# CliMA/ClimateParameterizations.jl

Hardware: AMD Instinct MI355X
Metric: column-timesteps/sec (fwd+adjoint), 32-level wind-mixing NDE (higher is better)
Workload: dtype f32

## Files before the change

### climateparameterizations.jl_amd/csrc/engine_regtile.hip

```cpp
#include <cstdlib>
#include "engine_regtile.h"
#include "kernel_select.h"
#include "split_bf16.h"

typedef float f32x16 __attribute__((ext_vector_type(16)));

#ifdef COLNDE_STAMPS
__device__ unsigned long long g_rt_stamps[16];
#define RT_STAMP_DECL unsigned long long rs_t0 = 0, rs_acc[8] = {0, 0, 0, 0, 0, 0, 0, 0}; const unsigned long long rs_kk = __builtin_amdgcn_s_memtime(), rs_rr = __builtin_amdgcn_s_memrealtime()
#define RT_STAMP_BEGIN() do { __builtin_amdgcn_sched_barrier(0); rs_t0 = __builtin_amdgcn_s_memtime(); __builtin_amdgcn_sched_barrier(0); } while (0)
#define RT_STAMP(i) do { __builtin_amdgcn_sched_barrier(0); unsigned long long t_ = __builtin_amdgcn_s_memtime(); rs_acc[i] += t_ - rs_t0; rs_t0 = t_; __builtin_amdgcn_sched_barrier(0); } while (0)
#define RT_STAMP_FLUSH() do { if (blockIdx.x == 0 && threadIdx.x == 0) { for (int q_ = 0; q_ < 8; q_++) g_rt_stamps[q_] = rs_acc[q_]; g_rt_stamps[8] = __builtin_amdgcn_s_memtime() - rs_kk; g_rt_stamps[9] = __builtin_amdgcn_s_memrealtime() - rs_rr; } } while (0)
#else
#define RT_STAMP_DECL
#define RT_STAMP_BEGIN()
#define RT_STAMP(i)
#define RT_STAMP_FLUSH()
#endif
typedef float f32x4v __attribute__((ext_vector_type(4)));
typedef float f32x2v __attribute__((ext_vector_type(2)));

#define RHO0(r) (((r) & 3) + 8 * ((r) >> 2))
#ifndef RT16_WAVES
#define RT16_WAVES 8
#endif
#ifndef RT_ADJ_CH
#define RT_ADJ_CH 8
#endif
#ifndef RT_ZRICH
#define RT_ZRICH 0
#endif
#ifndef RT_Z2TAPE
#define RT_Z2TAPE 0
#endif
#define RT_TAPEZ_HALF (21 * 256)
#define RT_Z2OFF ((RT_ZRICH ? 2 : 1) * RT_TAPEZ_HALF)
#define RT_TAPEZ (RT_Z2OFF + (RT_Z2TAPE ? 9 * 256 : 0))
#define RT_TAPE2 (20 * 256)

__device__ __forceinline__ f32x16 mfma32(float a, float b, f32x16 c) {
    return __builtin_amdgcn_mfma_f32_32x32x2f32(a, b, c, 0, 0, 0);
}

__device__ __forceinline__ float xchg32(float from_hi, float from_lo, int h) {
    const auto r = __builtin_amdgcn_permlane32_swap(__float_as_uint(from_hi), __float_as_uint(from_lo), false, false);
    return __uint_as_float(h ? r[0] : r[1]);
}
__device__ __forceinline__ float swap32(float x, int h) { return xchg32(x, x, h); }

__device__ __forceinline__ f32x16 shift_down(const f32x16 T, int h, float below) {
    f32x16 o;
#pragma unroll
    for (int g = 0; g < 4; g++) {
        const float recv = xchg32(g > 0 ? T[(4 * g + 15) & 15] : 0.0f, T[4 * g + 3], h);
        o[4 * g] = (h == 0 && g == 0) ? below : recv;
        o[4 * g + 1] = T[4 * g];
        o[4 * g + 2] = T[4 * g + 1];
        o[4 * g + 3] = T[4 * g + 2];
    }
    return o;
}

__device__ __forceinline__ f32x16 shift_up(const f32x16 T, int h, float above) {
    f32x16 o;
#pragma unroll
    for (int g = 0; g < 4; g++) {
        const float recv = xchg32(T[4 * g], g < 3 ? T[(4 * g + 4) & 15] : 0.0f, h);
        o[4 * g + 3] = (h == 1 && g == 3) ? above : recv;
        o[4 * g] = T[4 * g + 1];
        o[4 * g + 1] = T[4 * g + 2];
        o[4 * g + 2] = T[4 * g + 3];
    }
    return o;
}

template <int ACT>
__device__ __forceinline__ float rt_act(float z) {
    if (ACT == COLNDE_ACT_RELU) return fmaxf(z, 0.0f);
    if (ACT == COLNDE_ACT_MISH) {
        const float e = __expf(__builtin_amdgcn_fmed3f(z, -3.0e38f, 20.0f));
        const float n = e * (e + 2.0f);
        return z * fast_div(n, n + 2.0f);
    }
    if (ACT == COLNDE_ACT_SWISH) return fast_div(z, 1.0f + __expf(-z));
    if (ACT == COLNDE_ACT_TANH) { const float e = __expf(2.0f * fminf(fmaxf(z, -15.0f), 15.0f)); return 1.0f - fast_div(2.0f, 1.0f + e); }
    if (ACT == COLNDE_ACT_LEAKYRELU) return z > 0.0f ? z : 0.01f * z;
    return z;
}

template <int ACT>
__device__ __forceinline__ f32x16 act_tile(f32x16 z) {
    f32x16 o;
#pragma unroll
    for (int r = 0; r < 16; r++) o[r] = rt_act<ACT>(z[r]);
    return o;
}

struct RtBases {
    int a1[5];
    int a2;
    int a3;
};

__device__ __forceinline__ RtBases rt_bases(int lane) {
    const int i = lane & 31, h = lane >> 5;
    const int r_i = (i & 3) + 4 * (i >> 3), h_i = (i >> 2) & 1;
    RtBases b;
#pragma unroll
    for (int mt = 0; mt < 5; mt++) {
        const int G = min(mt * 16 + r_i, 74);
// ... 513 lines not shown
    float av, dv;
    rt_act_pair<ACT>(A[G >> 4][G & 15], av, dv);
    A[G >> 4][G & 15] = av;
    D[G >> 4][G & 15] = dv;
}

__device__ __forceinline__ void rt_physics_vjp(const DevModel& m, const f32x16 (&X)[3], f32x16 (&kd)[3], int h, f32x16 (&xb)[3]) {
    const float Nz = 32.0f;
#pragma unroll
    for (int r = 0; r < 16; r++) {
        xb[0][r] = -m.cor_v * m.sig_u * kd[1][r];
        xb[1][r] = m.cor_u * m.sig_v * kd[0][r];
        xb[2][r] = 0.0f;
    }
#pragma unroll
    for (int k = 0; k < 3; k++) {
        const f32x16 dn = shift_down(kd[k], h, 0.0f);
#pragma unroll
        for (int r = 0; r < 16; r++) kd[k][r] = (r == 0 && h == 0) ? 0.0f : m.A[k] * (kd[k][r] - dn[r]);
    }
    if (!m.mpp && !m.ca) return;
    f32x16 gb[3];
    if (m.mpp) {
        const f32x16 Ud = shift_down(X[0], h, 0.0f), Vd = shift_down(X[1], h, 0.0f), Td = shift_down(X[2], h, 0.0f);
        const float cU = m.sig_u * Nz, sU = m.sig_u * m.eps, cV = m.sig_v * Nz, sV = m.sig_v * m.eps, cB = m.B * Nz, sB = m.B * m.eps;
        const float L2E = 1.4426950408889634f;
        const float kE = 2.0f * m.inv_dRi * L2E, oE = -2.0f * m.Ric * m.inv_dRi * L2E, cE = 30.0f * L2E;
        const float nA = -0.5f * m.nu_minus, nB = m.nu0 + 0.5f * m.nu_minus;
        const float m0 = -m.cs[0], m1 = -m.cs[1], m2 = -m.cs[2] * m.inv_Pr;
        const float n0 = m0 * Nz * m.c_rib, n1 = m1 * Nz * m.c_rib, n2 = m2 * Nz * m.c_rib;
        const float q0 = -2.0f * m.sig_u, q1 = -2.0f * m.sig_v;
#pragma unroll
        for (int r = 0; r < 16; r++) {
            const bool in = !(r == 0 && h == 0);
            const float dU = X[0][r] - Ud[r], dV = X[1][r] - Vd[r], dT = X[2][r] - Td[r];
            const float a1 = fmaf(dU, cU, sU), a2 = fmaf(dV, cV, sV);
            const float rS = __builtin_amdgcn_rcpf(fmaf(a2, a2, a1 * a1));
            const float Ri = fmaf(dT, cB, sB) * rS;
            const float e = __builtin_amdgcn_exp2f(__builtin_amdgcn_fmed3f(fmaf(Ri, kE, oE), -cE, cE));
            const float th = fmaf(-2.0f, __builtin_amdgcn_rcpf(1.0f + e), 1.0f);
            const float nu = fmaf(th, nA, nB);
            const float t0 = kd[0][r] * nu, t1 = kd[1][r] * nu, t2 = kd[2][r] * nu;
            float nub = (kd[0][r] * dU) * n0;
            nub = fmaf(kd[1][r] * dV, n1, nub);
            nub = fmaf(kd[2][r] * dT, n2, nub);
            const float w = nub * (fmaf(-th, th, 1.0f) * rS);
            const float qq = w * Ri;
            const float g2 = fmaf(w, m.B, t2 * m2);
            const float g0 = fmaf(qq, a1 * q0, t0 * m0);
            const float g1 = fmaf(qq, a2 * q1, t1 * m1);
            gb[0][r] = in ? g0 : 0.0f;
            gb[1][r] = in ? g1 : 0.0f;
            gb[2][r] = in ? g2 : 0.0f;
        }
    } else {
        const f32x16 Td = shift_down(X[2], h, 0.0f);
#pragma unroll
        for (int r = 0; r < 16; r++) {
            const bool in = !(r == 0 && h == 0);
            const float gT = (X[2][r] - Td[r]) * Nz;
            gb[0][r] = 0.0f;
            gb[1][r] = 0.0f;
            gb[2][r] = (in && gT < 0.0f) ? -kd[2][r] * m.cs[2] * m.kappa : 0.0f;
        }
    }
#pragma unroll
    for (int k = 0; k < 3; k++) {
        const f32x16 gu_ = shift_up(gb[k], h, 0.0f);
#pragma unroll
        for (int r = 0; r < 16; r++) xb[k][r] += (gb[k][r] - gu_[r]) * Nz;
    }
}

#define RT_DMA_AUX 2
#ifdef RT_PLAIN_TAPE_STORES
#define RT_NT_STORE4(p, v) (*reinterpret_cast<f32x4v*>(p) = (f32x4v)(v))
#define RT_NT_STORE1(p, v) (*(float*)(p) = (float)(v))
#else
#define RT_NT_STORE4(p, v) __builtin_nontemporal_store((f32x4v)(v), reinterpret_cast<f32x4v*>(p))
#define RT_NT_STORE1(p, v) __builtin_nontemporal_store((float)(v), (float*)(p))
#endif
#define RT_TAPE_LOAD4(p) __builtin_nontemporal_load(reinterpret_cast<const f32x4v*>(p))
#define RT_TB (32 * 36)
#define RT_LAM(e, lane) ((((e) >> 2) * 64 + (lane)) * 4 + ((e) & 3))
__device__ __forceinline__ f32x16 rt_transpose(float* tb, const f32x16 T, int wbase, int rbase) {
#pragma unroll
    for (int a = 0; a < 4; a++)
        *reinterpret_cast<f32x4v*>(tb + wbase + 8 * a) = (f32x4v){T[4 * a], T[4 * a + 1], T[4 * a + 2], T[4 * a + 3]};
    f32x16 o;
#pragma unroll
    for (int s = 0; s < 16; s++) o[s] = tb[rbase + 72 * s];
    return o;
}

__device__ __forceinline__ f32x16 rt_outer(f32x16 acc, const f32x16 TA, const f32x16 TB) {
#pragma unroll
    for (int s = 0; s < 16; s++) acc = mfma32(TA[s], TB[s], acc);
    return acc;
}

struct Bf3x2 { Bf3 b[2]; };
__device__ __forceinline__ Bf3x2 rt_split_tile(const f32x16 T) {
    Bf3x2 o;
#pragma unroll
    for (int b = 0; b < 2; b++) {
        float v[8];
#pragma unroll
        for (int u = 0; u < 8; u++) v[u] = T[8 * b + u];
        o.b[b] = bf3_split8(v);
    }
    return o;
}
__device__ __forceinline__ f32x16 rt_outer_split(f32x16 acc, const Bf3x2& A, const Bf3x2& B) {
    acc = mfma_bf3(A.b[0], B.b[0], acc);
    acc = mfma_bf3(A.b[1], B.b[1], acc);
    return acc;
}

__device__ __forceinline__ float rt_sum16(const f32x16 v) {
    float s = 0.0f;
#pragma unroll
    for (int r = 0; r < 16; r++) s += v[r];
    return s;
}

#define RT_NET_LO(mt) (((mt) * 16) / 25)
#define RT_NET_HI(mt) ((((mt) * 16 + 15) < 75 ? ((mt) * 16 + 15) : 74) / 25)
__host__ __device__ constexpr int rt_combo(int n, int mt) { return n == 0 ? mt : (n == 1 ? 1 + mt : 2 + mt); }

template <int ACT, bool ZT, bool SPLIT = false>
__global__ void __launch_bounds__(256)
rt_adjoint_kernel(DevModel m, const float* __restrict__ wimg, const float* __restrict__ bcs,
                  const float* __restrict__ save_times, int n_save, int substeps, const float* __restrict__ sol,
                  const float* __restrict__ truth, const float* __restrict__ tape, float* __restrict__ tape2,
                  const float* __restrict__ tapez ,
                  LossWeights lw, float* __restrict__ slab, int n_col) {
    static_assert(!SPLIT || ZT, "the split W1^T operands replace the fp32 W1 in LDS: no layer-1 recomputation");
    float* wl = rt_smem;
    if constexpr (SPLIT) {
        static_assert(RT_ASIMG_HM_WORDS + 576 <= RT_W2C, "the split W1^T operands must fit the fp32 W1's place");
        const u32x4* src = reinterpret_cast<const u32x4*>(wimg + RT_ASIMG_OFF);
        for (int e = threadIdx.x; e < (RT_ASIMG_HM_WORDS + 576) / 4; e += blockDim.x) reinterpret_cast<u32x4*>(rt_smem)[e] = src[e];
        for (int e = RT_W2C + threadIdx.x; e < RT_IMG_FLOATS; e += blockDim.x) wl[e] = wimg[e];
    } else {
        for (int e = threadIdx.x; e < RT_IMG_FLOATS; e += blockDim.x) wl[e] = wimg[e];
    }
    __syncthreads();
    const int lane = threadIdx.x & 63, wave = threadIdx.x >> 6;
    const int j = lane & 31, h = lane >> 5;
    const int tile = blockIdx.x * RT_WAVES + wave;
    if (tile * RT_COLS >= n_col) return;
    float* lam = rt_smem + ((RT_IMG_FLOATS + 3) & ~3) + wave * (3072 + RT_TB);
    float* tb = lam + 3072;
    const int col = tile * RT_COLS + j;
    const bool valid = col < n_col;
    const int i_ = lane & 31, r_i = (i_ & 3) + 4 * (i_ >> 3), h_i = (i_ >> 2) & 1;
    int a1n[2];
#pragma unroll
    for (int t = 0; t < 2; t++) a1n[t] = RT_W1C + (2 * min(t * 16 + r_i, 24) + h_i) * RT_LD1 + 4 * h;
    const int a2b = RT_W2C + ((r_i < 10) ? 2 * r_i + h_i : 0) * RT_LD2 + h;
    const int f2c = (r_i < 10) ? 2 * r_i + h_i : 20;
    const int b3T = RT_W3C + (4 * h - 1) * RT_LD3 + f2c;
    int b2T[2];
#pragma unroll
    for (int t = 0; t < 2; t++) b2T[t] = RT_W2C + h * RT_LD2 + ((t * 16 + r_i < 25) ? 2 * (t * 16 + r_i) + h_i : 50);
    const int b1T = RT_W1C + h * RT_LD1 + i_;
    const int wbase = j * 36 + 4 * h, rbase = h * 36 + i_;

    f32x16 gW3[3], gW2[3][2];
#pragma unroll
    for (int q = 0; q < 3; q++) { gW3[q] = (f32x16)(0.0f); gW2[q][0] = (f32x16)(0.0f); gW2[q][1] = (f32x16)(0.0f); }
    float b2acc[3] = {0, 0, 0}, b3acc[3] = {0, 0, 0};
    float sums[6] = {0, 0, 0, 0, 0, 0};
    RT_STAMP_DECL;
    f32x16 xb[3], X[3];
#pragma unroll
    for (int q = 0; q < 3; q++) xb[q] = (f32x16)(0.0f);
    f32x16 xbs[3];
#pragma unroll
    for (int q = 0; q < 3; q++) xbs[q] = (f32x16)(0.0f);
#pragma unroll
    for (int e = 0; e < 48; e++) lam[RT_LAM(e, lane)] = 0.0f;

    const int n_steps = (n_save - 1) * substeps;
    const float* tp = tape + (size_t)tile * n_steps * 4 * 3072 + lane * 4;
    float* tp2 = tape2 + (size_t)tile * n_steps * 4 * RT_TAPE2 + lane * 4;
    const float* tpz = ZT ? tapez + (size_t)tile * n_steps * 4 * RT_TAPEZ + lane * 4 : nullptr;

    auto inject = [&](int n, bool add) {
#pragma unroll
        for (int q = 0; q < 3; q++) {
            f32x16 d;
#pragma unroll
            for (int g = 0; g < 4; g++) {
                const size_t o = ((size_t)min(col, n_col - 1) * n_save + n) * 96 + q * 32 + 8 * g + 4 * h;
                const f32x4v a = *reinterpret_cast<const f32x4v*>(sol + o);
                const f32x4v b = *reinterpret_cast<const f32x4v*>(truth + o);
#pragma unroll
                for (int e = 0; e < 4; e++) d[4 * g + e] = valid ? a[e] - b[e] : 0.0f;
            }
            const f32x16 dd = shift_down(d, h, 0.0f);
            f32x16 gg;
#pragma unroll
            for (int r = 0; r < 16; r++) {
                gg[r] = (r == 0 && h == 0) ? 0.0f : (d[r] - dd[r]) * 32.0f;
                sums[q] += d[r] * d[r];
                sums[3 + q] += gg[r] * gg[r];
            }
            if (add) {
                const f32x16 gu_ = shift_up(gg, h, 0.0f);
#pragma unroll
                for (int r = 0; r < 16; r++)
                    lam[RT_LAM(q * 16 + r, lane)] += 2.0f * lw.w[q] * d[r] + 2.0f * lw.w[3 + q] * 32.0f * (gg[r] - gu_[r]);
            }
        }
    };
    inject(0, false);

    auto load_z1 = [&](int step, int st, int n, f32x16 (&Z)[2], f32x16 (&Dz)[2]) {
        size_t rec = (size_t)step * 4 + st;
#ifdef RT_ABL_Z1_CACHED
        { int z_ = 0; asm volatile("" : "+v"(z_)); rec = (size_t)z_; }
#endif
        const float* srcz = tpz + rec * RT_TAPEZ + n * 7 * 256;
#pragma unroll
        for (int grp = 0; grp < 7; grp++) {
            const f32x4v v = RT_TAPE_LOAD4(srcz + grp * 256);
#pragma unroll
            for (int e = 0; e < 4; e++)
                if (4 * grp + e < 25) Z[grp >> 2][(grp & 3) * 4 + e] = v[e];
        }
        if (RT_ZRICH) {
#pragma unroll
            for (int grp = 0; grp < 7; grp++) {
                const f32x4v v = RT_TAPE_LOAD4(srcz + RT_TAPEZ_HALF + grp * 256);
#pragma unroll
                for (int e = 0; e < 4; e++)
                    if (4 * grp + e < 25) Dz[grp >> 2][(grp & 3) * 4 + e] = v[e];
            }
        }
    };

    auto load_z2 = [&](int step, int st, int n, f32x16& Z) {
        const float* srcz = tpz + ((size_t)step * 4 + st) * RT_TAPEZ + RT_Z2OFF + n * 3 * 256;
#pragma unroll
        for (int grp = 0; grp < 3; grp++) {
            const f32x4v v = RT_TAPE_LOAD4(srcz + grp * 256);
#pragma unroll
            for (int e = 0; e < 4; e++) Z[4 * grp + e] = (4 * grp + e < 10) ? v[e] : 0.0f;
        }
#pragma unroll
        for (int r = 12; r < 16; r++) Z[r] = 0.0f;
    };

    auto load_x = [&](int step, int st) {
        const float* src = tp + ((size_t)step * 4 + st) * 3072;
#pragma unroll
        for (int q = 0; q < 3; q++)
#pragma unroll
            for (int g = 0; g < 4; g++) {
                const f32x4v v = RT_TAPE_LOAD4(src + (q * 4 + g) * 256);
                X[q][4 * g] = v[0]; X[q][4 * g + 1] = v[1]; X[q][4 * g + 2] = v[2]; X[q][4 * g + 3] = v[3];
            }
    };

    for (int iv = n_save - 2; iv >= 0; iv--) {
        const float dt = (save_times[iv + 1] - save_times[iv]) / (float)substeps;
        inject(iv + 1, true);
        for (int s = substeps - 1; s >= 0; s--) {
            const int step = iv * substeps + s;
#pragma nounroll
            for (int st = 3; st >= 0; st--) {
                const float cwl = (st == 0 || st == 3) ? dt / 6.0f : dt / 3.0f;
                const float cwx = st == 3 ? 0.0f : (st == 2 ? dt : 0.5f * dt);
                RT_STAMP_BEGIN();
                f32x16 A1[2], D1[2];
                f32x16 A1n[2], D1n[2];
#pragma unroll
                for (int r = 9; r < 16; r++) { A1[1][r] = 0.0f; D1[1][r] = 0.0f; A1n[1][r] = 0.0f; D1n[1][r] = 0.0f; }
                load_x(step, st);
                f32x16 dOk[3];
                {
                    f32x16 kb[3];
#pragma unroll
                    for (int q = 0; q < 3; q++)
#pragma unroll
                        for (int r = 0; r < 16; r++) kb[q][r] = cwl * lam[RT_LAM(q * 16 + r, lane)] + cwx * xb[q][r];
                    rt_physics_vjp(m, X, kb, h, xb);
#pragma unroll
                    for (int q = 0; q < 3; q++) dOk[q] = kb[q];
                }
                RT_STAMP(0);
                float* dst = tp2 + ((size_t)step * 4 + st) * RT_TAPE2;
                float carry[2] = {0.0f, 0.0f};
#pragma unroll
                for (int n = 0; n < 3; n++) {
                    const f32x16 dOn = dOk[n];
                    if (ZT) {
                        if (n == 0) {
                            load_z1(step, st, 0, A1, D1);
#ifdef COLNDE_STAMPS
                            asm volatile("s_waitcnt vmcnt(0)" ::: "memory");
                            RT_STAMP(7);
#endif
                            if (!RT_ZRICH) {
#pragma unroll
                                for (int G = 0; G < 24; G += 4) rt_act_pair4_at<ACT>(A1, D1, G);
                                rt_act_pair_at<ACT>(A1, D1, 24);
                            }
                        }
                    } else {
#pragma unroll
                        for (int t = 0; t < 2; t++) {
                            f32x16 acc;
#pragma unroll
                            for (int r = 0; r < 16; r++) acc[r] = (t * 16 + r < 25) ? wl[RT_B1C + n * 50 + 2 * (t * 16 + r) + h] : 0.0f;
                            const int base = a1n[t] + n * 50 * RT_LD1;
                            acc = rt_chain<48, RT_ADJ_CH>(wl, acc, [=](int k) { return base + (k >> 4) * 32 + RHO0(k & 15); },
                                                          [&](int k) { return X[k >> 4][k & 15]; });
#pragma unroll
                            for (int r = 0; r < 16; r++) {
                                float av = 0.0f, dv = 0.0f;
                                if (t * 16 + r < 25) rt_act_pair<ACT>(acc[r], av, dv);
                                A1[t][r] = av;
                                D1[t][r] = dv;
                            }
                        }
                    }
                    RT_STAMP(1);
                    f32x16 Z2;
                    if (ZT && RT_Z2TAPE) load_z2(step, st, n, Z2);
                    else {
                        f32x16 acc;
#pragma unroll
                        for (int r = 0; r < 16; r++) acc[r] = r < 10 ? wl[RT_B2C + n * 20 + 2 * r + h] : 0.0f;
                        const int base2 = a2b + n * 20 * RT_LD2;
                        Z2 = rt_chain<25, 5>(wl, acc, [=](int k) { return base2 + 2 * k; },
                                             [&](int k) { return A1[k >> 4][k & 15]; });
                    }
                    RT_STAMP(2);
                    {
#ifndef RT_ABL_NO_OUTER
                        const f32x16 TA = rt_transpose(tb, dOn, wbase, rbase);
                        b3acc[n] += rt_sum16(TA);
#endif
                        f32x16 A2;
#pragma unroll
                        for (int r = 0; r < 16; r += 4) {
                            f32x2v a0 = {0.0f, 0.0f}, d0 = {0.0f, 0.0f}, a1 = {0.0f, 0.0f}, d1 = {0.0f, 0.0f};
                            if (r < 8) rt_act_pair4<ACT>((f32x2v){Z2[r], Z2[r + 1]}, (f32x2v){Z2[r + 2], Z2[r + 3]}, a0, d0, a1, d1);
                            else if (r == 8) rt_act_pair2<ACT>((f32x2v){Z2[8], Z2[9]}, a0, d0);
                            A2[r] = a0.x; A2[r + 1] = a0.y; A2[r + 2] = a1.x; A2[r + 3] = a1.y;
                            Z2[r] = d0.x; Z2[r + 1] = d0.y; Z2[r + 2] = d1.x; Z2[r + 3] = d1.y;
                        }
#ifndef RT_ABL_NO_OUTER
                        const f32x16 TB = rt_transpose(tb, A2, wbase, rbase);
#ifdef RT_OUTER_SPLIT
                        if constexpr (SPLIT) gW3[n] = rt_outer_split(gW3[n], rt_split_tile(TA), rt_split_tile(TB));
                        else
#endif
                        gW3[n] = rt_outer(gW3[n], TA, TB);
#else
                        gW3[n][0] += A2[0];
#endif
                    }
                    {
                        const int base = b3T + n * 31 * RT_LD3;
                        const f32x16 da = rt_chain<16, 8>(wl, (f32x16)(0.0f), [=](int k) { return base + RHO0(k) * RT_LD3; },
                                                          [&](int k) { return dOn[k]; });
#pragma unroll
                        for (int r = 0; r < 16; r++) Z2[r] = da[r] * Z2[r];
                    }
                    RT_STAMP(3);
                    if (ZT && n < 2) load_z1(step, st, n + 1, A1n, D1n);
#ifndef RT_LPIPE
#define RT_LPIPE 1
#endif
                    u32x4 Lr[9];
                    const u32x4* lg = nullptr;
                    if constexpr (SPLIT) {
                        int lz = lane;
                        asm volatile("" : "+v"(lz));
                        lg = reinterpret_cast<const u32x4*>(wimg + RT_ASIMG_OFF + RT_ASIMG_L) + n * 9 * 64 + lz;
#pragma unroll
                        for (int u = 0; u < (RT_LPIPE ? 3 : 9); u++) Lr[u] = lg[u * 64];
                    }
#ifdef RT_ABL_NO_OUTER
                    gW2[n][0][0] += Z2[0] * A1[0][0]; gW2[n][1][0] += Z2[1] * A1[1][0];
#else
                    {
                        const f32x16 TA = rt_transpose(tb, Z2, wbase, rbase);
                        b2acc[n] += rt_sum16(TA);
#ifdef RT_OUTER_SPLIT
                        Bf3x2 TAs;
                        if constexpr (SPLIT) TAs = rt_split_tile(TA);
#endif
#pragma unroll
                        for (int t = 0; t < 2; t++) {
                            const f32x16 TB = rt_transpose(tb, A1[t], wbase, rbase);
#ifdef RT_OUTER_SPLIT
                            if constexpr (SPLIT) gW2[n][t] = rt_outer_split(gW2[n][t], TAs, rt_split_tile(TB));
                            else
#endif
                            gW2[n][t] = rt_outer(gW2[n][t], TA, TB);
                        }
                    }
#endif
                    RT_STAMP(4);
#pragma unroll
                    for (int t = 0; t < 2; t++) {
                        const int base = b2T[t] + n * 20 * RT_LD2;
                        const f32x16 da = rt_chain<10, 10>(wl, (f32x16)(0.0f), [=](int k) { return base + 2 * k * RT_LD2; },
                                                           [&](int k) { return Z2[k]; });
#pragma unroll
                        for (int r = 0; r < 16; r++) D1[t][r] = da[r] * D1[t][r];
                    }
                    auto store_delta = [&] {
#pragma unroll
                    for (int g = 0; g < 25; g++) {
                        const int G = 25 * n + g;
                        if ((G & 3) == 0 && g + 3 < 25) {
                            const f32x4v v = {D1[g >> 4][g & 15], D1[(g + 1) >> 4][(g + 1) & 15], D1[(g + 2) >> 4][(g + 2) & 15],
                                              D1[(g + 3) >> 4][(g + 3) & 15]};
                            RT_NT_STORE4(dst + (G >> 2) * 256, v);
                        }
                    }
                    if (n == 0) carry[0] = D1[1][8];
                    if (n == 1) {
                        RT_NT_STORE4(dst + 6 * 256, ((f32x4v){carry[0], D1[0][0], D1[0][1], D1[0][2]}));
                        carry[0] = D1[1][7];
                        carry[1] = D1[1][8];
                    }
                    if (n == 2) {
                        RT_NT_STORE4(dst + 12 * 256, ((f32x4v){carry[0], carry[1], D1[0][0], D1[0][1]}));
                        RT_NT_STORE4(dst + 18 * 256, ((f32x4v){D1[1][6], D1[1][7], D1[1][8], 0.0f}));
                    }
                    };
#ifndef RT_ABL_NO_TAPE2
                    if constexpr (!SPLIT) store_delta();
#endif
                    RT_STAMP(5);
                    if constexpr (SPLIT) {
                        const u32x4* hm = reinterpret_cast<const u32x4*>(rt_smem) + lane;
#pragma unroll
                        for (int c = 0; c < 3; c++) {
                            if (RT_LPIPE && c < 2) {
#pragma unroll
                                for (int u = 0; u < 3; u++) Lr[3 * (c + 1) + u] = lg[(3 * (c + 1) + u) * 64];
                            }
                            float d8[8];
#pragma unroll
                            for (int u = 0; u < 8; u++) d8[u] = D1[(8 * c + u) >> 4][(8 * c + u) & 15];
                            const Bf3 Bc = bf3_split8(d8);
#pragma unroll
                            for (int q = 0; q < 3; q++) {
                                const int G = n * 9 + c * 3 + q, slot = c * 3 + q;
                                const u32x4 Ah = hm[(G * 2) * 64], Am = hm[(G * 2 + 1) * 64];
                                if (ZT && !RT_ZRICH && n < 2 && slot >= 2) {
                                    if (slot < 8) rt_act_pair4_at<ACT>(A1n, D1n, 4 * (slot - 2));
                                    else rt_act_pair_at<ACT>(A1n, D1n, 24);
                                }
                                xb[q] = mfma_bf(Am, Bc.m, xb[q]);
                                xb[q] = mfma_bf(Ah, Bc.l, xb[q]);
                                xb[q] = mfma_bf(Am, Bc.h, xb[q]);
                                xb[q] = mfma_bf(Ah, Bc.m, xb[q]);
                                xb[q] = mfma_bf(Ah, Bc.h, xb[q]);
                                xb[q] = mfma_bf(Lr[slot], Bc.h, xb[q]);
                                RT_SCHED_FENCE();
                            }
                        }
                        const float* left = rt_smem + RT_ASIMG_LEFT + (n * 2 + h) * 96 + i_;
#pragma unroll
                        for (int q = 0; q < 3; q++) xb[q] = mfma32(left[q * 32], D1[1][8], xb[q]);
                        store_delta();
                    } else
#pragma unroll
                    for (int q = 0; q < 3; q++) {
                        const int base = b1T + q * 32 + n * 50 * RT_LD1;
                        xb[q] = rt_chain_fill<25, 5>(wl, xb[q], [=](int g) { return base + 2 * g * RT_LD1; },
                                                     [&](int g) { return D1[g >> 4][g & 15]; },
                                                     [&](int c) {
                                                         if (ZT && !RT_ZRICH && n < 2 && (q > 0 || c > 0)) {
#pragma unroll
                                                             for (int G = 0; G < 24; G += 4)
                                                                 if ((G >> 2) * 2 + 2 == q * 5 + c)
                                                                     rt_act_pair4_at<ACT>(A1n, D1n, G);
                                                             if (q * 5 + c == 14) rt_act_pair_at<ACT>(A1n, D1n, 24);
                                                         }
                                                     });
                    }
                    if (ZT && n < 2) {
#pragma unroll
                        for (int t = 0; t < 2; t++) { A1[t] = A1n[t]; D1[t] = D1n[t]; }
                    }
                }
                RT_STAMP(6);
#pragma unroll
                for (int q = 0; q < 3; q++) xbs[q] += xb[q];
            }
#pragma unroll
            for (int q = 0; q < 3; q++) {
#pragma unroll
                for (int r = 0; r < 16; r++) lam[RT_LAM(q * 16 + r, lane)] += xbs[q][r];
                xbs[q] = (f32x16)(0.0f);
            }
        }
    }

#ifndef COLNDE_STAMPS_FWD
    RT_STAMP_FLUSH();
#endif
    float* out = slab + (size_t)tile * (m.n_params + 8);
    const int r_j = (j & 3) + 4 * (j >> 3), h_j = (j >> 2) & 1;
#pragma unroll
    for (int n = 0; n < 3; n++) {
        if (r_j < 10) {
            const int f2 = 2 * r_j + h_j;
#pragma unroll
            for (int r = 0; r < 16; r++) {
                const int face = RHO0(r) + 4 * h;
                if (face >= 1) out[n * m.net_size + m.w_off[2] + f2 * 31 + face - 1] = gW3[n][r];
            }
        }
#pragma unroll
        for (int t = 0; t < 2; t++) {
            const int Gp = t * 16 + r_j;
            if (Gp < 25) {
                const int f1 = 2 * Gp + h_j;
#pragma unroll
                for (int r = 0; r < 10; r++) out[n * m.net_size + m.w_off[1] + f1 * 20 + 2 * r + h] = gW2[n][t][r];
            }
        }
        const float s2 = b2acc[n] + swap32(b2acc[n], h), s3 = b3acc[n] + swap32(b3acc[n], h);
        if (h == 0) {
            if (r_i < 10) out[n * m.net_size + m.b_off[1] + 2 * r_i + h_i] = s2;
            if (i_ >= 1) out[n * m.net_size + m.b_off[2] + i_ - 1] = s3;
        }
    }
#pragma unroll
    for (int q = 0; q < 6; q++) {
        float v = sums[q];
        for (int off = 32; off > 0; off >>= 1) v += __shfl_down(v, off);
        if (lane == 0) out[m.n_params + q] = v;
    }
}

#define RT_DW1_LDS (4 * 2048)
__global__ void __launch_bounds__(256)
rt_dw1_kernel(DevModel m, const float* __restrict__ tape, const float* __restrict__ tape2, long n_items,
              float* __restrict__ slab_rows) {
    const int lane = threadIdx.x & 63, wave = __builtin_amdgcn_readfirstlane(threadIdx.x >> 6);
    const int j = lane & 31, h = lane >> 5;
    float* buf = rt_smem + wave * RT_DW1_LDS;
    const long gw = (long)blockIdx.x * RT_WAVES + wave, GW = (long)gridDim.x * RT_WAVES;
    f32x16 gW1[5][3];
#pragma unroll
    for (int mt = 0; mt < 5; mt++)
#pragma unroll
        for (int q = 0; q < 3; q++) gW1[mt][q] = (f32x16)(0.0f);
    float b1acc[5] = {0, 0, 0, 0, 0};
    const int NQ = gw < n_items ? 4 * (int)((n_items - gw + GW - 1) / GW) : 0;
    const int soff = ((lane >> 1) & 3) * 256 + ((lane & 1) * 32 + (lane >> 3)) * 4;
    auto issue = [&](int Q, int ring) {
        const int Qc = Q < NQ ? Q : NQ - 1;
        const size_t item = (size_t)(gw + (long)(Qc >> 2) * GW);
        const float* sx = tape + item * 3072 + soff + (Qc & 3) * 32;
        const float* sz = tape2 + item * RT_TAPE2 + soff + (Qc & 3) * 32;
#pragma unroll
        for (int T = 0; T < 3; T++) __builtin_amdgcn_global_load_lds(sx + T * 1024, buf + ring * 2048 + T * 256, 16, 0, RT_DMA_AUX);
#pragma unroll
        for (int T = 0; T < 5; T++) __builtin_amdgcn_global_load_lds(sz + T * 1024, buf + ring * 2048 + (3 + T) * 256, 16, 0, RT_DMA_AUX);
    };
    const float* rd = buf + h * 32 + j;
    float op[2][8][4];
    auto read_set = [&](int set, int ring) {
#pragma unroll
        for (int T = 0; T < 8; T++)
#pragma unroll
            for (int s = 0; s < 4; s++) op[set][T][s] = rd[ring * 2048 + T * 256 + 64 * s];
    };
    if (NQ > 0) {
        issue(0, 0);
        issue(1, 1);
        issue(2, 2);
        asm volatile("s_waitcnt vmcnt(16)" ::: "memory");
        read_set(0, 0);
    }
    for (int Qb = 0; Qb < NQ; Qb += 4) {
#pragma unroll
        for (int u = 0; u < 4; u++) {
            const int cur = u & 1;
// ... 2091 lines not shown
                    for (int i = 0; i < 11; i++) *reinterpret_cast<f32x4v*>(rec + rec_wr[i]) = *reinterpret_cast<const f32x4v*>(stg + stg_rd[i]);
                }
#pragma unroll
                for (int t = 0; t < 4; t++) gb1[t] += dZ1[t];
#pragma unroll
                for (int u = 0; u < 2; u++) { gb2[u] += dZ2[u]; gb3[u] += dO.t[u]; }
                RT_STAMP(3);
                if constexpr (SPLIT) {
                    const float d80[8] = {dZ1[0][0], dZ1[0][1], dZ1[0][2], dZ1[0][3], dZ1[1][0], dZ1[1][1], dZ1[1][2], dZ1[1][3]};
                    const float d81[8] = {dZ1[2][0], dZ1[2][1], dZ1[2][2], dZ1[2][3], dZ1[3][0], dZ1[3][1], dZ1[3][2], dZ1[3][3]};
                    const Bf3 B0 = bf3_split8(d80);
                    Bf3 B1 = B0;
                    f32x4t c2[6];
#pragma unroll
                    for (int tl = 0; tl < 6; tl++) {
                        Bf3 A0;
                        A0.h = Hm[tl * 2 + 0]; A0.m = Hm[tl * 2 + 1]; A0.l = Lr[tl];
                        c2[tl] = mfma16_bf3(A0, B0, (f32x4t)(0.0f));
                        RT_SCHED_FENCE();
                        if (tl < 4) {
                            bf3_split_pair(d81[2 * tl], d81[2 * tl + 1], tl, B1);
                            RT_SCHED_FENCE();
                        }
                    }
#pragma unroll
                    for (int tl = 0; tl < 6; tl++) {
                        Bf3 A1_;
                        A1_.h = Hm[(6 + tl) * 2 + 0]; A1_.m = Hm[(6 + tl) * 2 + 1]; A1_.l = Lr[6 + tl];
                        c2[tl] = mfma16_bf3(A1_, B1, c2[tl]);
                        ex[(n * 6 + tl) * 64 + lane] = c2[tl];
                        RT_SCHED_FENCE();
                    }
                } else
#pragma unroll
                for (int q = 0; q < 3; q++) {
                    if (q < 2) rt16_fetch_ops<2, 13>(wl, a1[(q + 1) & 1], [&](int c, int k) { return b1T + 32 * (q + 1) + 16 * c + 4 * k * RT_LD1; });
                    RT_SCHED_HARD();
                    f32x4t c2[2] = {(f32x4t)(0.0f), (f32x4t)(0.0f)};
                    rt16_run_ops<2, 13>(a1[q & 1], c2, [&](int k) { return dZ1[k >> 2][k & 3]; });
#pragma unroll
                    for (int tau = 0; tau < 2; tau++) ex[(n * 6 + q * 2 + tau) * 64 + lane] = c2[tau];
                    RT_SCHED_HARD();
                }
                RT_STAMP(4);
                asm volatile("s_waitcnt lgkmcnt(0)\n\ts_barrier" ::: "memory");
                RT_STAMP(5);
            }
        }
    }
#ifndef COLNDE_STAMPS_FWD
    RT_STAMP_FLUSH();
#endif
    auto colsum = [&](float v) {
        v += __shfl_xor(v, 1); v += __shfl_xor(v, 2); v += __shfl_xor(v, 4); v += __shfl_xor(v, 8);
        return v;
    };
#pragma unroll
    for (int Q = 0; Q < 13; Q++) {
        const float v = colsum(gb1[Q >> 2][Q & 3]);
        if (j == 0 && (Q < 12 || g < 2)) out[n * m.net_size + m.b_off[0] + 4 * Q + g] = v;
    }
#pragma unroll
    for (int Q2 = 0; Q2 < 5; Q2++) {
        const float v = colsum(gb2[Q2 >> 2][Q2 & 3]);
        if (j == 0) out[n * m.net_size + m.b_off[1] + 4 * Q2 + g] = v;
    }
#pragma unroll
    for (int v_ = 0; v_ < 2; v_++)
#pragma unroll
        for (int r = 0; r < 4; r++) {
            const float v = colsum(gb3[v_][r]);
            const int face = 16 * v_ + 4 * g + r;
            if (j == 0 && face >= 1) out[n * m.net_size + m.b_off[2] + face - 1] = v;
        }
}

bool rt_supported(const DevModel& m) {
    return m.model == COLNDE_MODEL_WIND_MIXING && m.Nz == 32 && m.n_layers == 3 && m.sizes[0] == 96 && m.sizes[1] == 50 &&
           m.sizes[2] == 20 && m.sizes[3] == 31 && m.acts[0] == m.acts[1] && m.acts[2] == COLNDE_ACT_IDENTITY &&
           !m.smooth_NN && !m.smooth_Ri && !m.inplace;
}

size_t rt_forward_lds_bytes() { return (size_t)RT_IMG_FLOATS * sizeof(float); }
size_t rt_adjoint_lds_bytes() { return ((size_t)((RT_IMG_FLOATS + 3) & ~3) + RT_WAVES * (3072 + RT_TB)) * sizeof(float); }
static constexpr size_t rt_pad4(size_t floats) { return (floats + 3) & ~(size_t)3; }
static constexpr size_t RT_IMG_BYTES = rt_pad4(RT_IMG_FLOATS) * sizeof(float);
static constexpr size_t RT16S_FWD_XCH = 3 * 2 * 64 * 16;
static constexpr size_t RT16S_ADJ_XCH = 3 * 6 * 64 * 16;
static constexpr size_t RT16S_ADJ_STG = 3 * RT16S_STG * sizeof(float);
static size_t rt16_forward_lds_bytes(bool split) { return split ? ((size_t)RT_SIMG_WORDS + (RT_IMG_FLOATS - RT_B1C)) * sizeof(float) : rt_forward_lds_bytes(); }
static size_t rt16s_forward_lds_bytes() { return RT_IMG_BYTES + 2 * RT16S_FWD_XCH; }
static size_t rt16sh_forward_lds_bytes(bool split) {
    return (split ? ((size_t)RT_SIMG2_WORDS + rt_pad4(RT_IMG_FLOATS - RT_W3C)) * sizeof(float) : RT_IMG_BYTES) + 3 * RT16S_FWD_XCH;
}
static size_t rt16s_adjoint_lds_bytes() { return RT_IMG_BYTES + 2 * RT16S_ADJ_XCH + RT16S_ADJ_STG; }
static size_t rt16sh_adjoint_lds_bytes(bool split) {
    const size_t rest = RT16S_ADJ_XCH + 3 * 2 * 64 * 16 + RT16S_ADJ_STG;
    return split ? rt_pad4(RT_IMG_FLOATS - RT_W2C) * sizeof(float) + rest + (size_t)RT_NSA_HM_WORDS * 4 : RT_IMG_BYTES + rest;
}
static size_t rt_dw1_lds_bytes() { return RT_WAVES * RT_DW1_LDS * sizeof(float); }
size_t rt_tape_floats(int n_col, int n_steps) { return (size_t)((n_col + RT_COLS - 1) / RT_COLS) * n_steps * 4 * 3072; }
size_t rt_tape2_floats(int n_col, int n_steps) { return (size_t)((n_col + RT_COLS - 1) / RT_COLS) * n_steps * 4 * RT_TAPE2; }
size_t rt_split_rich_record_floats() { return RT16S_RREC; }
size_t rt_tapez_floats(int n_col, int n_steps) { return (size_t)((n_col + RT_COLS - 1) / RT_COLS) * n_steps * 4 * RT_TAPEZ; }
int rt_n_wtiles(int n_col) { return (n_col + RT_COLS - 1) / RT_COLS; }
int rt_dw1_waves(int n_col, int n_steps) {
    const long items = (long)rt_n_wtiles(n_col) * n_steps * 4;
    const long w = items < 1024 ? items : 1024;
    return (int)((w + RT_WAVES - 1) / RT_WAVES) * RT_WAVES;
}

using RtForwardFn = decltype(&rt_forward_kernel<COLNDE_ACT_RELU>);
using Rt16ForwardFn = decltype(&rt16_forward_kernel<COLNDE_ACT_RELU, false>);
using Rt16sForwardFn = decltype(&rt16s_forward_kernel<COLNDE_ACT_RELU, false>);
using Rt16shForwardFn = decltype(&rt16sh_forward_kernel<COLNDE_ACT_RELU, false>);
using Rt16sAdjointFn = decltype(&rt16s_adjoint_kernel<COLNDE_ACT_RELU, false>);
using Rt16shAdjointFn = decltype(&rt16sh_adjoint_kernel<COLNDE_ACT_RELU, false>);
using RtAdjointFn = decltype(&rt_adjoint_kernel<COLNDE_ACT_RELU, false>);

static RtForwardFn rt_forward_pick(int act) {
    RtForwardFn k = nullptr;
    with_act(act, [&](auto A) { k = rt_forward_kernel<decltype(A)::value>; });
    return k;
}
static Rt16ForwardFn rt16_forward_pick(int act, bool split) {
    Rt16ForwardFn k = nullptr;
    with_act(act, [&](auto A) { with_bools([&](auto S) { k = rt16_forward_kernel<decltype(A)::value, decltype(S)::value>; }, split); });
    return k;
}
static Rt16sForwardFn rt16s_forward_pick(int act, bool rich) {
    Rt16sForwardFn k = nullptr;
    with_act(act, [&](auto A) { with_bools([&](auto R) { k = rt16s_forward_kernel<decltype(A)::value, decltype(R)::value>; }, rich); });
    return k;
}
static Rt16shForwardFn rt16sh_forward_pick(int act, bool rich, bool rkc, bool split) {
    Rt16shForwardFn k = nullptr;
    with_act(act, [&](auto A) {
        with_bools([&](auto R, auto K, auto S) { k = rt16sh_forward_kernel<decltype(A)::value, decltype(R)::value, decltype(K)::value, decltype(S)::value>; }, rich, rkc, split);
    });
    return k;
}
static Rt16sAdjointFn rt16s_adjoint_pick(int act, bool rich) {
    Rt16sAdjointFn k = nullptr;
    with_act(act, [&](auto A) { with_bools([&](auto R) { k = rt16s_adjoint_kernel<decltype(A)::value, decltype(R)::value>; }, rich); });
    return k;
}
static Rt16shAdjointFn rt16sh_adjoint_pick(int act, bool rich, bool rkc, bool split) {
    Rt16shAdjointFn k = nullptr;
    with_act(act, [&](auto A) {
        with_bools([&](auto R, auto K, auto S) { k = rt16sh_adjoint_kernel<decltype(A)::value, decltype(R)::value, decltype(K)::value, decltype(S)::value>; }, rich, rkc, split);
    });
    return k;
}
static RtAdjointFn rt_adjoint_pick(int act, bool ztape, bool split) {
    RtAdjointFn k = nullptr;
    with_act(act, [&](auto A) {
        with_bools([&](auto Z, auto S) {
            if constexpr (decltype(Z)::value || !decltype(S)::value) k = rt_adjoint_kernel<decltype(A)::value, decltype(Z)::value, decltype(S)::value>;
        }, ztape, split);
    });
    return k;
}
static auto rt_dw1_pick(bool split) { return split ? rt_dw1_split_kernel : rt_dw1_kernel; }

hipError_t rt_set_attributes() {
    hipError_t e = hipSuccess;
    const size_t v = 160 * 1024;
// ... 128 lines not shown
```

Before: 185.2 million.

## Stream Z1 tape records into LDS via async global_load_lds ring with vmcnt pacing

Replaces the register-destined nontemporal loads of the layer-1 Z tape in the adjoint kernel with asynchronous global-to-LDS DMA (global_load_lds). Four groups go to a per-wave LDS ring and the rest into the transposition tile. Waits on vmcnt are placed so the loads for the next record overlap the current chain computation. This is meant to hide tape-load latency and free VGPRs, at the cost of extra LDS per wave (a static assert checks the 160KB fit), a possible occupancy reduction, and fragile hand-counted vmcnt thresholds.

Result: no change. 186.4 million (median of 6 runs) (+0.7%).

```diff
diff --git a/climateparameterizations.jl_amd/csrc/engine_regtile.hip b/climateparameterizations.jl_amd/csrc/engine_regtile.hip
--- a/climateparameterizations.jl_amd/csrc/engine_regtile.hip
+++ b/climateparameterizations.jl_amd/csrc/engine_regtile.hip
@@ -26,6 +26,9 @@
 #endif
 #ifndef RT_ADJ_CH
 #define RT_ADJ_CH 8
+#endif
+#ifndef RT_LPIPE
+#define RT_LPIPE 1
 #endif
 #ifndef RT_ZRICH
 #define RT_ZRICH 0
@@ -705,6 +708,19 @@
 #endif
 #define RT_TAPE_LOAD4(p) __builtin_nontemporal_load(reinterpret_cast<const f32x4v*>(p))
 #define RT_TB (32 * 36)
+#ifndef RT_Z1_GLOBAL_LOADS
+#define RT_Z1_GLOBAL_LOADS 0
+#endif
+#if !RT_Z1_GLOBAL_LOADS && !RT_ZRICH && !defined(RT_ABL_Z1_CACHED) && !defined(RT_ABL_NO_TAPE2)
+#define RT_Z1_DMA 1
+#else
+#define RT_Z1_DMA 0
+#endif
+#define RT_Z1_RING 4
+#define RT_ADJ_LDS_FLOATS (((RT_IMG_FLOATS + 3) & ~3) + RT_WAVES * (3072 + RT_TB + RT_Z1_DMA * RT_Z1_RING * 256))
+static_assert(RT_ADJ_LDS_FLOATS * 4 <= 160 * 1024, "the adjoint kernel's LDS: image, lambda, transposition tiles and Z1 rings must fit one CU");
+static_assert(RT_Z1_RING <= 7 && (7 - RT_Z1_RING) * 256 <= RT_TB, "the rest of a Z1 record must fit the transposition tile");
+#define RT_VMCNT(n) asm volatile("s_waitcnt vmcnt(%0)" ::"n"(n) : "memory")
 #define RT_LAM(e, lane) ((((e) >> 2) * 64 + (lane)) * 4 + ((e) & 3))
 __device__ __forceinline__ f32x16 rt_transpose(float* tb, const f32x16 T, int wbase, int rbase) {
 #pragma unroll
@@ -775,6 +791,8 @@
     if (tile * RT_COLS >= n_col) return;
     float* lam = rt_smem + ((RT_IMG_FLOATS + 3) & ~3) + wave * (3072 + RT_TB);
     float* tb = lam + 3072;
+    [[maybe_unused]] float* zr = rt_smem + ((RT_IMG_FLOATS + 3) & ~3) + RT_WAVES * (3072 + RT_TB) + __builtin_amdgcn_readfirstlane(wave) * (RT_Z1_RING * 256);
+    [[maybe_unused]] float* ztb = rt_smem + ((RT_IMG_FLOATS + 3) & ~3) + __builtin_amdgcn_readfirstlane(wave) * (3072 + RT_TB) + 3072;
     const int col = tile * RT_COLS + j;
     const bool valid = col < n_col;
     const int i_ = lane & 31, r_i = (i_ & 3) + 4 * (i_ >> 3), h_i = (i_ >> 2) & 1;
@@ -840,7 +858,7 @@
     };
     inject(0, false);
 
-    auto load_z1 = [&](int step, int st, int n, f32x16 (&Z)[2], f32x16 (&Dz)[2]) {
+    [[maybe_unused]] auto load_z1 = [&](int step, int st, int n, f32x16 (&Z)[2], f32x16 (&Dz)[2]) {
         size_t rec = (size_t)step * 4 + st;
 #ifdef RT_ABL_Z1_CACHED
         { int z_ = 0; asm volatile("" : "+v"(z_)); rec = (size_t)z_; }
@@ -864,6 +882,26 @@
         }
     };
 
+    [[maybe_unused]] auto z1_dma = [&](long rec, int n, int g0, int g1) {
+        const float* srcz = tpz + (size_t)(rec < 0 ? 0 : rec) * RT_TAPEZ + n * 7 * 256;
+        asm volatile("" ::: "memory");
+#pragma unroll
+        for (int grp = 0; grp < 7; grp++)
+            if (grp >= g0 && grp < g1)
+                __builtin_amdgcn_global_load_lds(srcz + grp * 256, grp < RT_Z1_RING ? zr + grp * 256 : ztb + (grp - RT_Z1_RING) * 256, 16, 0, RT_DMA_AUX);
+        asm volatile("" ::: "memory");
+    };
+    [[maybe_unused]] auto z1_lds = [&](int grp, f32x16 (&Z)[2]) {
+        const f32x4v v = *reinterpret_cast<const f32x4v*>((grp < RT_Z1_RING ? zr + grp * 256 : tb + (grp - RT_Z1_RING) * 256) + lane * 4);
+#pragma unroll
+        for (int e = 0; e < 4; e++)
+            if (4 * grp + e < 25) Z[grp >> 2][(grp & 3) * 4 + e] = v[e];
+    };
+    [[maybe_unused]] constexpr int Z1_TILE_GROUPS = 7 - RT_Z1_RING;
+    [[maybe_unused]] constexpr int Z1_N_RING = Z1_TILE_GROUPS + (SPLIT ? (RT_LPIPE ? 6 : 9) : 6);
+    [[maybe_unused]] constexpr int Z1_N_TILE = SPLIT ? (RT_LPIPE ? 6 : 0) : 6;
+    [[maybe_unused]] constexpr int Z1_N_TOP = (SPLIT && RT_LPIPE ? 6 : 0) + 7 + 12;
+
     auto load_z2 = [&](int step, int st, int n, f32x16& Z) {
         const float* srcz = tpz + ((size_t)step * 4 + st) * RT_TAPEZ + RT_Z2OFF + n * 3 * 256;
 #pragma unroll
@@ -887,6 +925,10 @@
             }
     };
 
+    if constexpr (ZT && RT_Z1_DMA) {
+        z1_dma((long)n_steps * 4 - 1, 0, 0, 7);
+        RT_VMCNT(0);
+    }
     for (int iv = n_save - 2; iv >= 0; iv--) {
         const float dt = (save_times[iv + 1] - save_times[iv]) / (float)substeps;
         inject(iv + 1, true);
@@ -921,10 +963,19 @@
                     const f32x16 dOn = dOk[n];
                     if (ZT) {
                         if (n == 0) {
+#if RT_Z1_DMA
+                            RT_VMCNT(Z1_N_TOP);
+#ifdef COLNDE_STAMPS
+                            RT_STAMP(7);
+#endif
+#pragma unroll
+                            for (int grp = 0; grp < 7; grp++) z1_lds(grp, A1);
+#else
                             load_z1(step, st, 0, A1, D1);
 #ifdef COLNDE_STAMPS
                             asm volatile("s_waitcnt vmcnt(0)" ::: "memory");
                             RT_STAMP(7);
+#endif
 #endif
                             if (!RT_ZRICH) {
 #pragma unroll
@@ -995,9 +1046,10 @@
                         for (int r = 0; r < 16; r++) Z2[r] = da[r] * Z2[r];
                     }
                     RT_STAMP(3);
+#if RT_Z1_DMA
+                    if constexpr (ZT) z1_dma(n < 2 ? (long)step * 4 + st : (long)step * 4 + st - 1, n < 2 ? n + 1 : 0, 0, RT_Z1_RING);
+#else
                     if (ZT && n < 2) load_z1(step, st, n + 1, A1n, D1n);
-#ifndef RT_LPIPE
-#define RT_LPIPE 1
 #endif
                     u32x4 Lr[9];
                     const u32x4* lg = nullptr;
@@ -1029,6 +1081,12 @@
                         }
                     }
 #endif
+#if RT_Z1_DMA
+                    if constexpr (ZT) {
+                        RT_SCHED_HARD();
+                        z1_dma(n < 2 ? (long)step * 4 + st : (long)step * 4 + st - 1, n < 2 ? n + 1 : 0, RT_Z1_RING, 7);
+                    }
+#endif
                     RT_STAMP(4);
 #pragma unroll
                     for (int t = 0; t < 2; t++) {
@@ -1079,6 +1137,13 @@
                             for (int q = 0; q < 3; q++) {
                                 const int G = n * 9 + c * 3 + q, slot = c * 3 + q;
                                 const u32x4 Ah = hm[(G * 2) * 64], Am = hm[(G * 2 + 1) * 64];
+#if RT_Z1_DMA
+                                if (ZT && n < 2 && slot >= 1 && slot <= 7) {
+                                    if (slot == 1) RT_VMCNT(Z1_N_RING);
+                                    if (slot == RT_Z1_RING + 1) RT_VMCNT(Z1_N_TILE);
+                                    z1_lds(slot - 1, A1n);
+                                }
+#endif
                                 if (ZT && !RT_ZRICH && n < 2 && slot >= 2) {
                                     if (slot < 8) rt_act_pair4_at<ACT>(A1n, D1n, 4 * (slot - 2));
                                     else rt_act_pair_at<ACT>(A1n, D1n, 24);
@@ -1103,6 +1168,13 @@
                         xb[q] = rt_chain_fill<25, 5>(wl, xb[q], [=](int g) { return base + 2 * g * RT_LD1; },
                                                      [&](int g) { return D1[g >> 4][g & 15]; },
                                                      [&](int c) {
+#if RT_Z1_DMA
+                                                         if (ZT && n < 2 && ((q * 5 + c) & 1)) {
+                                                             if (q * 5 + c == 1) RT_VMCNT(Z1_N_RING);
+                                                             if (q * 5 + c == 2 * RT_Z1_RING + 1) RT_VMCNT(Z1_N_TILE);
+                                                             z1_lds((q * 5 + c) >> 1, A1n);
+                                                         }
+#endif
                                                          if (ZT && !RT_ZRICH && n < 2 && (q > 0 || c > 0)) {
 #pragma unroll
                                                              for (int G = 0; G < 24; G += 4)
@@ -1130,6 +1202,7 @@
         }
     }
 
+    if constexpr (ZT && RT_Z1_DMA) RT_VMCNT(0);
 #ifndef COLNDE_STAMPS_FWD
     RT_STAMP_FLUSH();
 #endif
@@ -3387,7 +3460,7 @@
 }
 
 size_t rt_forward_lds_bytes() { return (size_t)RT_IMG_FLOATS * sizeof(float); }
-size_t rt_adjoint_lds_bytes() { return ((size_t)((RT_IMG_FLOATS + 3) & ~3) + RT_WAVES * (3072 + RT_TB)) * sizeof(float); }
+size_t rt_adjoint_lds_bytes() { return (size_t)RT_ADJ_LDS_FLOATS * sizeof(float); }
 static constexpr size_t rt_pad4(size_t floats) { return (floats + 3) & ~(size_t)3; }
 static constexpr size_t RT_IMG_BYTES = rt_pad4(RT_IMG_FLOATS) * sizeof(float);
 static constexpr size_t RT16S_FWD_XCH = 3 * 2 * 64 * 16;
```
